# tszalay/poreseq

Measured on AMD Instinct MI355X. Metric: kb consensus refined/sec at 10x coverage, higher is better.
Workload: dtype f64; 1 GPU; poreseq consensus, 10 kb region, 10x synthetic coverage (BASELINE configs[1]), full Mutate.py schedule per region; a step is 280 independent regions per GPU = 14 lock-step batches; the batches of the timed steps run step by step (a step's batches all finish before the next step's start) through 14 batch slots (host threads) per GPU; marshalling + H2D of the events, host greedy steps and D2H inside; region_bases=10000, events=10, regions_per_gpu=280, batches_in_flight=14, step_barrier=True, parallelism=280 regions x 1 GPU(s), 14 host thread(s) per GPU, no data-path collective

## Files before the change

poreseq_amd/csrc/ps_sweep.hip:

```cpp
#include "ps_sweep_body.h"

namespace ps {

__global__ __launch_bounds__(256) void k_band(BatchD b, SweepD sw) {
    const int jd = blockIdx.y, dir = jd % sw.ndir;
    const JobD& J = b.jobs[jd / sw.ndir];
    const SweepJob& SJ = sw.sj[jd];
    const int j = blockIdx.x * 256 + threadIdx.x;
    if (j > J.C + 1) return;
    int i0 = 0, i1 = J.n0;
    if (j > J.C) { i0 = J.n0 + 1; i1 = J.n0; }
    else if (j >= 1) band_of(b.lb + J.lb_off, dir, j, J.C, J.n0, J.W, i0, i1);
    sw.band[SJ.band_off + j] = make_int2(i0, i1);
}

__global__ __launch_bounds__(256) void k_qlo(BatchD b, SweepD sw) {
    const int jd = blockIdx.y;
    const JobD& J = b.jobs[jd / sw.ndir];
    const SweepJob& SJ = sw.sj[jd];
    const int t = blockIdx.x * 256 + threadIdx.x;
    int win = 0;
    if (t < SJ.T + Q_PAD) {
        const int K = sw.K, C = J.C;
        const int2* __restrict__ band = sw.band + SJ.band_off;
        int res = -1, top = -1;
        const int qa = max(0, t - C), qb = min(SJ.Q - 1, t - 1);
        if (t < SJ.T && qa <= qb && !J.out->inert) {
            int lo = qa, hi = qb + 1;
            while (lo < hi) { const int mid = (lo + hi) >> 1; if (band[t - mid].x <= mid * K + K) hi = mid; else lo = mid + 1; }
            if (lo <= qb && band[t - lo].y >= lo * K + 1) {
                res = lo;
                int l2 = lo, h2 = qb;
                while (l2 < h2) { const int mid = (l2 + h2 + 1) >> 1; if (band[t - mid].y >= mid * K + 1) l2 = mid; else h2 = mid - 1; }
                top = l2;
                win = l2 - lo + 1;
            }
        }
        sw.qlo[SJ.q_off + t] = res;
        sw.qhi[SJ.q_off + t] = top;
    }
    for (int off = 32; off; off >>= 1) win = max(win, __shfl_xor(win, off));
    if ((threadIdx.x & 63) == 0 && win > 0) atomicMax(sw.maxwin, win);
}

#define PS_SWEEP_WPE(K) K <= 10 ? 2 : 1

template <int K, bool FD>
__global__ __launch_bounds__(64) __attribute__((amdgpu_waves_per_eu(PS_SWEEP_WPE(K), PS_SWEEP_WPE(K))))
void k_sweep(BatchD b, SweepD sw) {
    __shared__ __attribute__((aligned(16))) char mring[mring_bytes(1)];
    const JobD& J = b.jobs[blockIdx.x];
    if (J.out->inert) return;
    sweep_body<K, 1, 0, 0, FD>(b, sw, J, sw.sj[blockIdx.x], nullptr, nullptr, mring);
}

template <int K, bool FD>
__global__ __launch_bounds__(64) __attribute__((amdgpu_waves_per_eu(PS_SWEEP_WPE(K), PS_SWEEP_WPE(K))))
void k_sweep2(BatchD b, SweepD sw) {
    __shared__ unsigned long long ring[ring_cols(1)];
    __shared__ __attribute__((aligned(16))) char mring[mring_bytes(1)];
    const int jd = blockIdx.x;
    const JobD& J = b.jobs[jd >> 1];
    if (J.out->inert) return;
    if ((jd & 1) == 0) sweep_body<K, 1, 0, 1, FD>(b, sw, J, sw.sj[jd], ring, nullptr, mring);
    else sweep_body<K, 1, 1, 1, FD>(b, sw, J, sw.sj[jd], ring, nullptr, mring);
}

template <int K, bool FD>
__global__ __launch_bounds__(64) __attribute__((amdgpu_waves_per_eu(PS_SWEEP_WPE(K), PS_SWEEP_WPE(K))))
void k_sweeps(BatchD b, SweepD sw) {
    __shared__ unsigned long long ring[ring_cols(1)];
    __shared__ __attribute__((aligned(16))) char mring[mring_bytes(1)];
    const int jd = blockIdx.x;
    const JobD& J = b.jobs[jd >> 1];
    if (J.out->inert) return;
    if ((jd & 1) == 0) sweep_body<K, 1, 0, 2, FD>(b, sw, J, sw.sj[jd], ring, nullptr, mring);
    else sweep_body<K, 1, 1, 2, FD>(b, sw, J, sw.sj[jd], ring, nullptr, mring);
}

__global__ __launch_bounds__(64) void k_best(BatchD b, SweepD sw) {
    chain_priority();
    const JobD& J = b.jobs[blockIdx.x];
    JobOut* O = J.out;
    if (O->inert) return;
    const SweepJob& SJ = sw.sj[blockIdx.x * sw.ndir];
    const StripBest* SB = sw.sb + SJ.sb_off;
    double v = 0.0;
    int bi = 0x7fffffff, bj = 0x7fffffff;
    for (int q = threadIdx.x; q < SJ.Q; q += 64) {
        const StripBest s = SB[q];
        if (s.v > v || (s.v == v && s.v > 0.0 && (s.j < bj || (s.j == bj && s.i < bi)))) { v = s.v; bi = s.i; bj = s.j; }
    }
    for (int off = 32; off; off >>= 1) {
        const double ov = __shfl_xor(v, off);
        const int oi = __shfl_xor(bi, off), oj = __shfl_xor(bj, off);
        if (ov > v || (ov == v && ov > 0.0 && (oj < bj || (oj == bj && oi < bi)))) { v = ov; bi = oi; bj = oj; }
    }
    if (threadIdx.x == 0) {
        O->best = v;
        if (v > 0.0) { O->bi = bi; O->bj = bj; } else { O->bi = 0; O->bj = 0; }
    }
}

template <int K>
struct StripCodes {
    const unsigned char* codes;
    const int2* band;
    const int* st;
    int nl;
    int ci0, ci1, cp0, cp1, cst;
    static constexpr bool ROWFAST = true;
    static constexpr bool TWO_PASS = true;
    __device__ __forceinline__ void prep(int, int tj, int t) {
        const int col = tj - (t & 63);
        ci0 = 1; ci1 = 0; cp0 = 0; cp1 = -1; cst = -1;
        if (col >= 1) {
            const int2 bc = band[col], bp = band[col - 1];
            ci0 = bc.x; ci1 = bc.y; cp0 = bp.x; cp1 = bp.y; cst = st[col - 1];
        }
    }
    __device__ __forceinline__ unsigned fetch(int ti, int tj, int a, int c) const {
        const int rs = max(ti - a, 1), col = max(tj - c, 1);
        const int q = (rs - 1) / K, rr = (rs - 1) - q * K;
        return code_fetch(codes + (size_t)(col + q) * (nl * K), K, q & (nl - 1), rr, nl);
    }
    __device__ __forceinline__ unsigned short decode(unsigned by, int ti, int tj, int a, int c) const {
        const int r = ti - a;
        const int cu = __builtin_amdgcn_readfirstlane(c);
        const int i0 = __builtin_amdgcn_readlane(ci0, cu), i1 = __builtin_amdgcn_readlane(ci1, cu);
        const int p0 = __builtin_amdgcn_readlane(cp0, cu), p1 = __builtin_amdgcn_readlane(cp1, cu);
        const int sc = __builtin_amdgcn_readlane(cst, cu);
        const bool cell = r >= 1 && tj - cu >= 1 && sc >= 0 && r >= i0 && r <= i1;
        const bool vd = r > p0 && r <= p1;
        const unsigned sm = code_main_step(by, vd), ss = code_stay_step(by);
        const unsigned w = sm | (ss << 8) | ((by & CB_POS) ? 0u : 0x4000u) | ((by & CB_SPOS) ? 0u : 0x8000u);
        return (unsigned short)(cell ? w : 0xC000u);
    }
};

template <int K>
__global__ __launch_bounds__(256) void k_backtrace_s(BatchD b, SweepD sw) {
    const JobD& J = b.jobs[blockIdx.x];
    const SweepJob& SJ = sw.sj[blockIdx.x * sw.ndir];
    StripCodes<K> src;
    src.codes = sw.codes + SJ.codes_off;
    src.band = sw.band + SJ.band_off;
    src.st = J.st;
    src.nl = sw.nl;
    bt_walk(J, src);
}

template <bool FD>
__device__ __forceinline__ double cell_emission(const BatchD& b, const JobD& J, int i, int j) {
    const int state = J.st[j - 1];
    const double2* row = (const double2*)((const char*)J.model8 + (size_t)max(state, 0) * MODEL_ROW_BYTES);
    const double2 q0 = row[0], q1 = row[1], q2 = row[2], q3 = row[3];
    const double m[8] = {q0.x, q0.y, q1.x, q1.y, q2.x, q2.y, q3.x, q3.y};
    const double4 l4 = ((const double4*)J.lev[0])[i - 1];
    const double lv[4] = {l4.x, l4.y, l4.z, l4.w};
    return emission8<FD>(m, lv, b.log2pi, J.lik_offset);
}

template <bool FD>
__global__ __launch_bounds__(256) void k_like_a(BatchD b) {
    const JobD& J = b.jobs[blockIdx.y];
    if (J.out->inert) return;
    const int t = blockIdx.x * 256 + threadIdx.x;
    if (t >= J.n0) return;
    const long long w = ((const long long*)J.rl)[t];
    double o = 0.0;
    if (w != 0) {
        const int j = (int)(w >> 4), st = (int)(w >> 1) & 7;
        if (st == (int)M_MATCH || st == (int)M_STAY || st == (int)M_EXTEND) o = cell_emission<FD>(b, J, t + 1, j);
    }
    J.ri[t] = o;
}

template <bool FD>
__global__ __launch_bounds__(64) void k_like_b(BatchD b) {
    chain_priority();
    const JobD& J = b.jobs[blockIdx.x];
    const JobOut O = *J.out;
    if (O.inert || O.bi <= 0) return;
    const int lane = threadIdx.x;
    const int iz = O.term_i, jz = O.term_w >> 3, kind = O.term_w & 3;
    const double lsk = J.lsk, lst = J.lst, lex = J.lex, lin = J.lin;
    double v = 0.0;
    if ((kind & 1) && iz >= 1 && jz >= 1) v = cell_emission<FD>(b, J, iz, jz);
    int curj = jz;
    long long* rlw = (long long*)J.rl;
    for (int i0 = iz + 1; i0 <= O.bi; i0 += 64) {
        const int i = i0 + lane;
        long long w = 0; double o = 0.0;
        if (i <= O.bi) { w = rlw[i - 1]; o = J.ri[i - 1]; }
        const int wj = (int)(w >> 4), wst = (int)(w >> 1) & 7;
        double res = 0.0;
        const int n = min(64, O.bi - i0 + 1);
        for (int k = 0; k < n; k++) {
            const int j = __builtin_amdgcn_readlane(wj, k), st = __builtin_amdgcn_readlane(wst, k);
            const double ok = __hiloint2double(__builtin_amdgcn_readlane(__double2hiint(o), k), __builtin_amdgcn_readlane(__double2loint(o), k));
            const int jx = (st == (int)M_MATCH || st == (int)M_IGNORE) ? j - 1 : j;
            for (int s = curj; s < jx; s++) v = v + lsk;
            if (st == (int)M_MATCH) v = v + ok;
            else if (st == (int)M_IGNORE || st == (int)M_INSERT) v = v + lin;
            else if (st == (int)M_STAY) v = v + ok + lst;
            else v = v + ok + lex;
            curj = j;
            res = lane == k ? v : res;
        }
        if (i <= O.bi) J.rl[i - 1] = res;
    }
}

constexpr int LK_MAXC = 12 * 1024;
__global__ __launch_bounds__(256) void k_likes(BatchD b, const LikeGroup* __restrict__ groups, double* __restrict__ out) {
    __shared__ int s_idx[LK_MAXC];
    __shared__ int s_part[256];
    const LikeGroup G = groups[blockIdx.x];
    const int tid = threadIdx.x, nk = G.C + 4;
    double* __restrict__ lk = out + G.out_off;
    const int chunk = (nk + 255) / 256, k0 = min(nk, tid * chunk), k1 = min(nk, k0 + chunk);
    for (int k = tid; k < G.len; k += 256) lk[k] = 0.0;
    for (int e = 0; e < G.njobs; e++) {
        const JobD& J = b.jobs[G.job0 + e];
        const double* __restrict__ ra = J.ra;
        const double* __restrict__ rl = J.rl;
        for (int k = tid; k < nk; k += 256) s_idx[k] = -1;
        __syncthreads();
        for (int t = tid; t < J.n0; t += 256) {
            const double a = ra[t];
            if (a > 0) { const int k = (int)a; if (k < nk) atomicMax(&s_idx[k], t); }
        }
        __syncthreads();
        int run = -1;
        for (int k = k0; k < k1; k++) { run = max(run, s_idx[k]); s_idx[k] = run; }
        s_part[tid] = run;
        __syncthreads();
        int before = -1;
        for (int q = 0; q < tid; q++) before = max(before, s_part[q]);
        for (int k = k0; k < k1; k++) {
            const int t = max(s_idx[k], before);
            if (k >= 1 && k < G.C + 3 && k + 1 < G.len) lk[k + 1] += t >= 0 ? rl[t] : 0.0;
        }
        __syncthreads();
    }
}

int launch_likes(Runtime* rt, const BatchD& b, const LikeGroup* d_groups, int ngroups, double* d_out) {
    if (!ngroups) return PS_OK;
    hipLaunchKernelGGL(k_likes, dim3(ngroups), dim3(256), 0, rt->stream, b, d_groups, d_out);
    PS_LAUNCH_CHECK();
    return PS_OK;
}
int likes_max_states() { return LK_MAXC - 4; }

struct SweepHeight { int K; bool on[3]; };
static const SweepHeight HEIGHTS[] = {
#define PS_X(K, W1, W2, W4) {K, {W1, W2, W4}},
    PS_SWEEP_HEIGHTS(PS_X)
#undef PS_X
};
template <class F>
static int first_height(int NW, F ok) {
    const int c = NW == 1 ? 0 : NW == 2 ? 1 : NW == 4 ? 2 : -1;
    for (const SweepHeight& h : HEIGHTS) if (c >= 0 && h.on[c] && ok(h.K)) return h.K;
    return 0;
}
int sweep_win_max(int NW) { return 64 * NW - 1; }
int sweep_guess_window(int W, int K) { return (2 * W + 1) / (K + 1) + 3; }

SweepForm sweep_guess_form(int W, int NW) {
    SweepForm f;
    f.K = first_height(NW, [&](int K) { return sweep_guess_window(W, K) <= sweep_win_max(NW); });
    if (f.K) f.NW = NW;
    return f;
}
SweepForm sweep_next_form(SweepForm f, int win) {
    SweepForm n;
    n.K = first_height(f.NW, [&](int K) { return K > f.K; });
    if (n.K) n.NW = f.NW;
    else if (f.NW > 1) n.K = first_height(1, [&](int K) { return K * sweep_win_max(1) > f.K * win; });
    return n;
}
bool sweep_form_exists(int K, int NW) { return first_height(NW, [&](int k) { return k == K; }) != 0; }
int sweep_guess_k(int W) { return sweep_guess_form(W, 1).K; }

template <int K>
static void sweep_launch_k(Runtime* rt, const BatchD& b, const SweepD& sw) {
    if (sw.ndir == 2 && sw.sparse) with_fastdiv(b.fastdiv, [&](auto fd) { hipLaunchKernelGGL((k_sweeps<K, fd.value>), dim3(b.njobs * 2), dim3(64), 0, rt->stream, b, sw); });
    else if (sw.ndir == 2) with_fastdiv(b.fastdiv, [&](auto fd) { hipLaunchKernelGGL((k_sweep2<K, fd.value>), dim3(b.njobs * 2), dim3(64), 0, rt->stream, b, sw); });
    else with_fastdiv(b.fastdiv, [&](auto fd) { hipLaunchKernelGGL((k_sweep<K, fd.value>), dim3(b.njobs), dim3(64), 0, rt->stream, b, sw); });
}

double sweep_job_bytes(int n0, int C, SweepForm f, bool full) {
    const int K = std::max(f.K, 1);
    const double steps = (double)C + (n0 + K - 1) / K + 1;
    return steps * 64.0 * f.NW * K * (full ? 1.0 + 2 * 16.0 : 1.0);
}

int sweep_prepare(Runtime* rt, Batch& bt, SweepForm f) {
    const BatchD& b = bt.d;
    const int nd = bt.ndir, K = f.K, NL = 64 * f.NW;
    std::vector<SweepJob>& sj = bt.sjobs;
    sj.resize(bt.jobs.size() * nd);
    int64_t band_tot = 0, q_tot = 0, sb_tot = 0, code_tot = 0, rec_tot = 0;
    int maxT = 0;
    for (size_t k = 0; k < bt.jobs.size(); k++) {
        JobD& j = bt.jobs[k];
        j.K = nd == 2 ? (bt.sparse ? -1 : K) : 0;
        j.NL = NL;
        if (bt.sparse) j.pitch = (std::min(2 * j.W + 1, j.n0) + 2 * (K - 1) + 3) & ~1;
        for (int d = 0; d < nd; d++) {
            SweepJob s;
            s.Q = (j.n0 + K - 1) / K;
            s.T = j.C + s.Q;
            s.band_off = band_tot; band_tot += j.C + 2;
            s.q_off = q_tot; q_tot += s.T + Q_PAD;
            s.sb_off = sb_tot; if (d == 0) sb_tot += std::max(s.Q, 1);
            s.codes_off = code_tot; if (d == 0) code_tot += (int64_t)s.T * NL * K;
            if (nd == 2 && bt.sparse) { j.mat_off[d] = rec_tot + (K - 1); rec_tot += (int64_t)bt.nkeep[2 * k + d] * j.pitch + 2 * K; }
            else if (nd == 2) { j.mat_off[d] = rec_tot; rec_tot += (int64_t)s.T * NL * K; }
            maxT = std::max(maxT, s.T);
            sj[k * nd + d] = s;
        }
    }
    bt.sweep_K = K; bt.sweep_NW = f.NW; bt.sweep_maxT = maxT; bt.sweep_code_bytes = code_tot; bt.sweep_sb = sb_tot; bt.sweep_recs = rec_tot;
    PS_TRY(rt->buf("sw_jobs").ensure(std::max<size_t>(sj.size(), 1) * sizeof(SweepJob)));
    PS_TRY(rt->buf("sw_band").ensure(std::max<int64_t>(band_tot, 1) * sizeof(int2)));
    PS_TRY(rt->buf("sw_qlo").ensure(std::max<int64_t>(q_tot, 1) * sizeof(int)));
    PS_TRY(rt->buf("sw_qhi").ensure(std::max<int64_t>(q_tot, 1) * sizeof(int)));
    PS_TRY(rt->buf("sw_sb").ensure(std::max<int64_t>(sb_tot, 1) * sizeof(StripBest)));
    PS_TRY(rt->buf("sw_win").ensure(64));
    PS_TRY(rt->up(rt->buf("sw_jobs").p, sj.data(), sj.size() * sizeof(SweepJob)));
    SweepD& sw = bt.sd;
    sw.sj = rt->buf("sw_jobs").as<SweepJob>();
    sw.band = rt->buf("sw_band").as<int2>();
    sw.qlo = rt->buf("sw_qlo").as<int>();
    sw.qhi = rt->buf("sw_qhi").as<int>();
    sw.sb = (StripBest*)rt->buf("sw_sb").p;
    sw.maxwin = rt->buf("sw_win").as<int>();
    sw.codes = nullptr;
    sw.K = K;
    sw.nl = NL;
    sw.ndir = nd;
    sw.sparse = nd == 2 && bt.sparse ? 1 : 0;
    PS_HIP(hipMemsetAsync(sw.maxwin, 0, sizeof(int), rt->stream));
    hipLaunchKernelGGL(k_band, dim3((bt.maxC + 2 + 255) / 256, b.njobs * nd), dim3(256), 0, rt->stream, b, sw);
    hipLaunchKernelGGL(k_qlo, dim3((maxT + Q_PAD + 255) / 256, b.njobs * nd), dim3(256), 0, rt->stream, b, sw);
    PS_LAUNCH_CHECK();
    return PS_OK;
}

int sweep_run(Runtime* rt, Batch& bt) {
    const BatchD& b = bt.d;
    SweepD& sw = bt.sd;
    const int K = bt.sweep_K, NW = bt.sweep_NW;
    if (!sweep_form_exists(K, NW)) return fail(PS_ERR_BAD_ARG, "sweep_run: no strip sweep of " + std::to_string(K) + " rows per lane on " + std::to_string(NW) + " wavefronts is built");
    PS_HIP(hipMemsetAsync(sw.sb, 0, (size_t)std::max<int64_t>(bt.sweep_sb, 1) * sizeof(StripBest), rt->stream));
    prof_begin(rt);
    if (NW > 1) {
        if (!b.fastdiv || !sweepw_launch(rt, b, sw, K, NW)) return fail(PS_ERR_BAD_ARG, "sweep_run: no such multi-wavefront form");
    } else {
        switch (K) {
#define PS_X(K, W1, W2, W4) PS_FORM_##W1(case K: sweep_launch_k<K>(rt, b, sw); break;)
            PS_SWEEP_HEIGHTS(PS_X)
#undef PS_X
        }
    }
    PS_LAUNCH_CHECK();
    prof_end(rt, "sweep", 0.0);
    if (rt->prof_on) {
        if (NW > 1) rt->prof[NW == 2 ? "sweep_w2" : "sweep_w4"].launches++;
        if (bt.ndir == 2 && bt.sparse) rt->prof["sweep_kept"].launches++;
        if (!b.fastdiv) rt->prof["sweep_ieee"].launches++;
    }
    hipLaunchKernelGGL(k_best, dim3(b.njobs), dim3(64), 0, rt->stream, b, sw);
    if (bt.ndir == 2) PS_TRY(launch_prefix(rt, b, 2));
    switch (K) {
#define PS_X(K, W1, W2, W4) case K: hipLaunchKernelGGL((k_backtrace_s<K>), dim3(b.njobs), dim3(256), 0, rt->stream, b, sw); break;
        PS_SWEEP_HEIGHTS(PS_X)
#undef PS_X
    }
    PS_LAUNCH_CHECK();
    if (bt.maxn > 0) {
        with_fastdiv(b.fastdiv, [&](auto fd) {
            hipLaunchKernelGGL(k_like_a<fd.value>, dim3((bt.maxn + 255) / 256, b.njobs), dim3(256), 0, rt->stream, b);
            hipLaunchKernelGGL(k_like_b<fd.value>, dim3(b.njobs), dim3(64), 0, rt->stream, b);
        });
        PS_LAUNCH_CHECK();
    }
    return PS_OK;
}

}
```

poreseq_amd/csrc/ps_sweep_body.h:

```cpp
#ifndef PS_SWEEP_BODY_H_
#define PS_SWEEP_BODY_H_

#include "ps_dev.h"
#include "ps_host.h"
#include "ps_codes.h"

namespace ps {

#ifdef __HIPCC__
__device__ __forceinline__ unsigned code_push(unsigned w, bool c) {
    const unsigned long long m = __builtin_amdgcn_ballot_w64(c);
    unsigned long long carry_out;
    asm("v_addc_co_u32_e64 %0, %1, %2, %2, %3" : "=v"(w), "=s"(carry_out) : "v"(w), "s"(m));
    return w;
}
__device__ __forceinline__ unsigned code_first(bool c) {
    const unsigned long long m = __builtin_amdgcn_ballot_w64(c);
    unsigned w;
    asm("v_cndmask_b32_e64 %0, 0, 1, %1" : "=v"(w) : "s"(m));
    return w;
}
#endif

struct StripBest { double v; int i, j; };
constexpr int Q_PAD = 8;

__device__ __forceinline__ double wave_ror1(double v) {
    int lo = __double2loint(v), hi = __double2hiint(v);
    lo = __builtin_amdgcn_update_dpp(lo, lo, 0x13C , 0xf, 0xf, false);
    hi = __builtin_amdgcn_update_dpp(hi, hi, 0x13C, 0xf, 0xf, false);
    return __hiloint2double(hi, lo);
}

__host__ __device__ constexpr int mring_slots(int nw) { return 128 * nw; }
__host__ __device__ constexpr int mring_bytes(int nw) { return (mring_slots(nw) + 1) * MODEL_ROW_BYTES; }

__host__ __device__ constexpr int ring_cols(int nw) { return nw <= 2 ? 256 : 512; }
constexpr int HAND_DOUBLES = 4;

template <int K, int NW, int DIR, int MODE, bool FD>
__device__ __forceinline__ void sweep_body(const BatchD& b, const SweepD& sw, const JobD& J, const SweepJob& SJ, unsigned long long* ring, double* hand, char* mring) {
    constexpr int NL = 64 * NW;
    constexpr int RING = ring_cols(NW);
    constexpr int RM = mring_slots(NW);
    const int lane = threadIdx.x;
    const int wv = NW > 1 ? uni((int)threadIdx.x >> 6) : 0;
    const int C = uni(J.C), T = uni(SJ.T), n0 = uni(J.n0);
    typedef const __attribute__((address_space(4))) int* kcip;
    kcip QLO = (kcip)uni_ptr(sw.qlo + SJ.q_off);
    kcip QHI = (kcip)uni_ptr(sw.qhi + SJ.q_off);
    gcip band = (gcip)uni_ptr((const int*)(sw.band + SJ.band_off));
    gcip st = (gcip)uni_ptr(J.st);
    const PS_GLOBAL char* model = (const PS_GLOBAL char*)uni_ptr((const char*)J.model8);
    const PS_GLOBAL v4d* levs = (const PS_GLOBAL v4d*)uni_ptr(J.lev[DIR]);
    PS_GLOBAL unsigned char* codes = (PS_GLOBAL unsigned char*)uni_ptr(sw.codes + SJ.codes_off);
    PS_GLOBAL char* rec = (PS_GLOBAL char*)uni_ptr((char*)(b.rec + J.mat_off[DIR]));
    PS_GLOBAL double* gcmax = (PS_GLOBAL double*)uni_ptr(b.cmax + J.col_off[DIR]);
    StripBest* SB = sw.sb + SJ.sb_off;
    const double lsk = J.lsk, lst = J.lst, lex = J.lex, lin = J.lin, off = J.lik_offset, log2pi = b.log2pi;
    const double NINF = -__builtin_inf();

    struct Ahead { int p1, i0, i1, sc, kc, ro; };
    gcip keep = (gcip)uni_ptr(J.keep[DIR]);
    const int pitch = uni(J.pitch);
    const PS_GLOBAL char* band_c = (const PS_GLOBAL char*)band;
    const PS_GLOBAL char* st_c = (const PS_GLOBAL char*)(DIR == 0 ? st - 1 : st);
    const PS_GLOBAL char* keep_c = (const PS_GLOBAL char*)keep;
    const PS_GLOBAL char* levs_c = (const PS_GLOBAL char*)levs;
    auto fetch = [&](int tt, int ql) -> Ahead {
        const int q = ql + ((lane - ql) & (NL - 1));
        const int j = clampi(tt - q, 1, max(C, 1));
        Ahead a;
        typedef int v3i_a4 __attribute__((ext_vector_type(3), aligned(4)));
        const v3i_a4 b3 = *(const PS_GLOBAL v3i_a4*)(band_c + (unsigned)(8 * j - 4));
        a.p1 = b3.x; a.i0 = b3.y; a.i1 = b3.z;
        a.sc = *(const PS_GLOBAL int*)(st_c + (unsigned)(4 * (DIR == 0 ? j : C - j)));
        a.kc = MODE == 2 ? *(const PS_GLOBAL int*)(keep_c + (unsigned)(4 * j)) : -1;
        a.ro = (j & (RM - 1)) * MODEL_ROW_BYTES;
        return a;
    };
    auto model_row = [&](const Ahead& a, double (&m)[8]) {
        const v2d* row = (const v2d*)(mring + a.ro);
        const v2d q0 = row[0], q1 = row[1], q2 = row[2], q3 = row[3];
        m[0] = q0.x; m[1] = q0.y; m[2] = q1.x; m[3] = q1.y; m[4] = q2.x; m[5] = q2.y; m[6] = q3.x; m[7] = q3.y;
    };

    const bool feeder = wv == 0;
    typedef const __attribute__((address_space(4))) int* kst_t;
    kst_t st_k = (kst_t)uni_ptr(J.st);
    int jf = 0;
    int fs0 = -1, fs1 = -1, fsb = -1;
    auto st_of = [&](int c) -> int { return st_k[DIR == 0 ? c - 1 : C - c]; };
    auto ring_at = [&](int c, int q16) -> v4i* { return (v4i*)(mring + (c <= C ? (c & (RM - 1)) : RM) * MODEL_ROW_BYTES + q16); };
    auto feed_now = [&](int hi) {
        const int fcol = (lane & 63) >> 2, fq16 = (lane & 3) * 16;
        const int lo = max(1, hi - (NL - 2));
        if (jf < lo - 1) jf = lo - 1;
        while (jf < hi) {
            const int c = jf + 1 + fcol, cc = min(c, max(C, 1));
            const int state = *(const PS_GLOBAL int*)(st_c + (unsigned)(4 * (DIR == 0 ? cc : C - cc)));
            const v4i row = *(const PS_GLOBAL v4i*)(model + (unsigned)max(state, 0) * (unsigned)MODEL_ROW_BYTES + (unsigned)fq16);
            *ring_at(c, fq16) = row;
            jf += 16;
        }
        fsb = -1;
    };
    v4i frow = {0, 0, 0, 0};
    bool fput = false;
    auto f_top = [&](int hi_next, int jn_now) {
        if (!feeder) return;
        if (hi_next > 0 && jf < min(C, hi_next)) feed_now(min(C, hi_next));
        fput = false;
        if (jf < C && fsb == jf && jn_now > 0 && jf + 2 <= jn_now + NL + 1) {
            if ((lane & 63) < 8) {
                const int state = (lane & 4) ? fs1 : fs0;
                frow = *(const PS_GLOBAL v4i*)(model + (unsigned)max(state, 0) * (unsigned)MODEL_ROW_BYTES + (unsigned)((lane & 3) * 16));
            }
            fput = true;
        }
    };
    auto f_end = [&]() {
        if (!feeder) return;
        if (fput) {
            if ((lane & 63) < 8) *ring_at(jf + 1 + ((lane & 4) >> 2), (lane & 3) * 16) = frow;
            jf += 2;
        }
        if (jf < C && fsb != jf) { fsb = jf; fs0 = st_of(min(jf + 1, C)); fs1 = st_of(min(jf + 2, C)); }
    };

    double lev[K][4];
    double pm[K];
    double pe[DIR ? K : 1];
#pragma unroll
    for (int r = 0; r < K; r++) { pm[r] = NINF; if (DIR) pe[r] = NINF; lev[r][0] = 0.0; lev[r][1] = 1.0; lev[r][2] = 0.0; lev[r][3] = 1.0; }
    int qcur = -1;
    double bot_m = NINF, bot_s = NINF, bot_e = NINF;
    double dm = NINF, de = NINF;
    double lbest = 0.0;
    int lbt = 0, lbr = 0;
    int flushed = 1, next_flush = 64;
    if (MODE) {
        for (int k = lane; k < RING; k += NL) ring[k] = 0ull;
    }
    const int pw = NW > 1 ? (wv + NW - 1) % NW : 0;
    const bool l0 = NW > 1 && (lane & 63) == 0, l63 = NW > 1 && (lane & 63) == 63;
    if (NW > 1) {
        if (l63) {
#pragma unroll
            for (int s = 0; s < 2; s++) { double* h = hand + (s * NW + wv) * HAND_DOUBLES; h[0] = NINF; h[1] = NINF; h[2] = NINF; }
        }
        asm volatile("s_waitcnt lgkmcnt(0)\n\ts_barrier" ::: "memory");
    }

    int ql0 = QLO[1], ql1 = QLO[2], ql2 = QLO[3];
    Ahead aA = fetch(1, ql0), aB = fetch(2, ql1), aC = aB;
    double mr[8];
    if (feeder) { feed_now(min(max(C, 1), ql0 >= 0 ? max(1 - ql0, 1) : 1)); if (jf < C) { fsb = jf; fs0 = st_of(min(jf + 1, C)); fs1 = st_of(min(jf + 2, C)); } }
    if (NW > 1) asm volatile("s_waitcnt lgkmcnt(0)\n\ts_barrier" ::: "memory");
    model_row(aA, mr);
    int qlev = -1;
    auto load_levels = [&](int ql_next) {
        if (ql_next < 0) return;
        const int qn = ql_next + ((lane - ql_next) & (NL - 1));
        if (qn != qlev) {
            qlev = qn;
#pragma unroll
            for (int r = 0; r < K; r++) {
                const v4d v = *(const PS_GLOBAL v4d*)(levs_c + (unsigned)(32 * min(qn * K + r, n0 - 1)));
                lev[r][0] = v.x; lev[r][1] = v.y; lev[r][2] = v.z; lev[r][3] = v.w;
            }
        }
    };
    load_levels(ql0);

    constexpr bool DEFER_REC = MODE == 2 && K <= 5;
    bool pend = false;
    unsigned cwp[(K + 3) / 4];
    double pnm[DEFER_REC ? K : 1], pns[DEFER_REC ? K : 1];
    bool pkept = false;
    unsigned poff = 0u;
#pragma unroll
    for (int w = 0; w < (K + 3) / 4; w++) cwp[w] = 0u;
    auto put_codes = [&](int tp, const unsigned (&cw)[(K + 3) / 4]) {
        PS_GLOBAL unsigned char* dst = codes + (size_t)tp * (NL * K);
        int r0 = 0;
#pragma unroll
        for (int g = 0; g < 8; g++) {
            const int sz = plane_sz(K - r0);
            PS_GLOBAL unsigned char* p = dst + (unsigned)(NL * r0 + lane * sz);
            if (sz == 16) {
                v4i v;
                v.x = cw[r0 / 4]; v.y = cw[r0 / 4 + 1]; v.z = cw[r0 / 4 + 2]; v.w = cw[r0 / 4 + 3];
                *(PS_GLOBAL v4i*)p = v;
            } else if (sz == 8) {
                typedef int v2i __attribute__((ext_vector_type(2)));
                v2i v;
                v.x = cw[r0 / 4]; v.y = cw[r0 / 4 + 1];
                *(PS_GLOBAL v2i*)p = v;
            } else if (sz == 4) {
                *(PS_GLOBAL unsigned*)p = cw[r0 / 4];
            } else {
                const int nrow = K - (r0 & ~3) < 4 ? K - (r0 & ~3) : 4;
                const int sh = CODE_BITS * (nrow - (r0 & 3) - sz);
                if (sz == 2) *(PS_GLOBAL unsigned short*)p = (unsigned short)(cw[r0 / 4] >> sh);
                else *p = (unsigned char)(cw[r0 / 4] >> sh);
            }
            r0 += sz;
            if (r0 >= K) break;
        }
    };
    auto put_pending = [&](int tp) {
        if (!pend) return;
        if (DIR == 0) put_codes(tp, cwp);
        if (DEFER_REC) {
            if (pkept) {
                PS_GLOBAL char* recp = rec - 16 * (K - 1) + poff;
#pragma unroll
                for (int r = 0; r < K; r++) *(PS_GLOBAL v2d*)(recp + r * 16) = (v2d){pnm[r], pns[r]};
            }
        }
    };

    auto step = [&](const int t, const Ahead& a0, const Ahead& a1, Ahead& a2) __attribute__((always_inline)) {
        const int ql = ql0;
        const bool live = ql >= 0;
        const int q = ql + ((lane - ql) & (NL - 1));
        const int j = t - q;
        if (live && q != qcur) {
            if (DIR == 0 && lbest > 0.0) { StripBest sbv; sbv.v = lbest; sbv.i = qcur * K + 1 + lbr; sbv.j = lbt - qcur; SB[qcur] = sbv; }
            lbest = 0.0;
            qcur = q;
#pragma unroll
            for (int r = 0; r < K; r++) { pm[r] = NINF; if (DIR) pe[r] = NINF; }
        }
        f_top(ql1 >= 0 ? t + 1 - ql1 : 0, ql >= 0 ? t - ql : 0);
        a2 = fetch(t + 2, ql2);
        __builtin_amdgcn_sched_barrier(0);
        double ov[K];
#pragma unroll
        for (int r = 0; r < K; r++) {
            ov[r] = emission8<FD>(mr, lev[r], log2pi, off);
            asm volatile("" : "+v"(ov[r]));
            if (r & 1) __builtin_amdgcn_sched_barrier(0);
        }
        __builtin_amdgcn_sched_barrier(0);
        double hm = NINF, hs = NINF, he = NINF;
        if (NW > 1) {
            asm volatile("s_waitcnt lgkmcnt(0)\n\ts_barrier" ::: "memory");
            const double* h = hand + (((t - 1) & 1) * NW + pw) * HAND_DOUBLES;
            const v2d hv = *(const v2d*)h;
            hm = hv.x; hs = hv.y;
            if (DIR) he = h[2];
        }
        put_pending(t - 1);
        load_levels(ql1);
        model_row(a1, mr);
        const int ql3 = QLO[t + 3];
        pend = live;
        if (MODE != 1 || live) {
            const int base = q * K + 1;
            const bool valid = live && j >= 1 && j <= C && a0.sc >= 0;
            const int ra = valid ? a0.i0 - base : K, rb = valid ? a0.i1 - base : -1;
            const int rp = a0.p1 - base;
            double um = wave_ror1(bot_m), us = wave_ror1(bot_s), ue = DIR ? wave_ror1(bot_e) : 0.0;
            if (NW > 1) { um = l0 ? hm : um; us = l0 ? hs : us; if (DIR) ue = l0 ? he : ue; }
            double dprev = dm, deprev = de;
            dm = um; de = ue;
            const double lbefore = lbest;
            double crun = 0.0;
            PS_GLOBAL char* recp = rec + ((size_t)t * K * NL + lane) * 16;
            const bool kept = MODE == 2 && live && a0.kc >= 0 && j >= 1 && j <= C;
            const bool kstore = kept && ra < K && rb >= 0;
            if (MODE == 2) {
                const unsigned ro = (unsigned)((a0.kc * pitch + (base - a0.i0) + (K - 1)) * 16);
                recp = rec - 16 * (K - 1) + ro;
                if (DEFER_REC) { poff = ro; pkept = kstore; }
                if (kept && !valid)
                    for (int r = max(0, a0.i0 - base); r <= min(K - 1, a0.i1 - base); r++) *(PS_GLOBAL v2d*)(recp + (size_t)r * 16) = (v2d){0.0, 0.0};
            }
            unsigned cw = 0u;
#pragma unroll
            for (int r = 0; r < K; r++) {
                const double o = ov[r];
                const bool act = r >= ra && r <= rb;
                const bool top = r == ra;
                const bool below = r - 1 >= ra && r <= rb;
                const double pmr = pm[r];
                double L;
                asm("v_max_f64 %0, %1, 0" : "=v"(L) : "v"(pmr));
                const bool blank = rp == r - 1;
                const double dq = __hiloint2double(blank ? (int)0xFFEFFFFF : __double2hiint(dprev), __double2loint(dprev));
                double D = dq;
                if (DIR == 0) asm("v_max_f64 %0, %1, 0" : "=v"(D) : "v"(dq));
                const double eq_ = DIR ? __hiloint2double(blank ? (int)0xFFEFFFFF : __double2hiint(deprev), __double2loint(deprev)) : 0.0;
                const double cSTAY = DIR == 0 ? um + o + lst : ue + lst;
                const double cEXT = DIR == 0 ? us + o + lex : us + lex;
                const double cINS = um + lin;
                const double cSKIP = L + lsk;
                const double cMATCH = DIR == 0 ? D + o : eq_;
                const double cIGN = dq + lin;
                const double floor_s = MODE == 1 ? (top ? -BIG : 0.0) : 0.0;
                const double t1 = fmax(floor_s, cSTAY);
                const double ns = fmax(t1, cEXT);
                double nm = fmax(0.0, cSKIP);
                nm = fmax(nm, cMATCH);
                nm = fmax(nm, cINS);
                nm = fmax(nm, cIGN);
                nm = fmax(nm, ns);
                if (DIR == 0) {
                    cw = (r & 3) == 0 ? code_first(cEXT > t1) : code_push(cw, cEXT > t1);
                    cw = code_push(cw, ns > 0.0);
                    cw = code_push(cw, cSKIP == nm);
                    cw = code_push(cw, cMATCH == nm);
                    cw = code_push(cw, cINS == nm);
                    cw = code_push(cw, cIGN == nm);
                    cw = code_push(cw, nm > 0.0);
                    if ((r & 3) == 3 || r == K - 1) cwp[r >> 2] = cw;
                }
                const double nmx = keep_or_absent(nm, act), nsx = keep_or_absent(ns, MODE == 1 ? act : below);
                dprev = pmr;
                pm[r] = nmx;
                if (DIR) { deprev = pe[r]; pe[r] = nmx + o; }
                um = nmx;
                us = DIR == 0 ? nsx : nsx + o;
                if (DIR) ue = nmx + o;
                if (MODE == 1) {
                    double rx;
                    asm("v_max_f64 %0, %1, 0" : "=v"(rx) : "v"(nmx));
                    *(PS_GLOBAL v2d*)(recp + (size_t)r * (16 * NL)) = (v2d){rx, act ? ns : 0.0};
                    crun = fmax(crun, rx);
                }
                if (MODE == 2) {
                    if (DEFER_REC) { pnm[r] = nmx; pns[r] = nsx; }
                    else if (kstore) *(PS_GLOBAL v2d*)(recp + r * 16) = (v2d){nmx, nsx};
                    crun = fmax(crun, nmx);
                }
                if (DIR == 0) {
                    const bool gt = nmx > lbest;
                    asm("v_max_f64 %0, %1, %2" : "=v"(lbest) : "v"(lbest), "v"(nmx));
                    lbr = gt ? r : lbr;
                }
                __builtin_amdgcn_sched_barrier(0);
            }
            bot_m = um; bot_s = us; bot_e = ue;
            if (DIR == 0) lbt = lbest > lbefore ? t : lbt;
            if (MODE) atomicMax(&ring[(unsigned)j & (RING - 1)], (unsigned long long)__double_as_longlong(crun));
            if (MODE && live && t >= next_flush) {
                const int jdone = min(t - QHI[t], C + 1);
                for (int col = flushed + lane; col < jdone; col += NL) {
                    unsigned long long* e = &ring[(unsigned)col & (RING - 1)];
                    const unsigned long long v = *e;
                    *e = 0ull;
                    gcmax[col] = __longlong_as_double((long long)v);
                }
                flushed = max(flushed, jdone);
                next_flush = t + 64;
            }
        } else {
            bot_m = NINF; bot_s = NINF; bot_e = NINF;
        }
        if (NW > 1 && l63) {
            double* h = hand + ((t & 1) * NW + wv) * HAND_DOUBLES;
            *(v2d*)h = (v2d){bot_m, bot_s};
            if (DIR) h[2] = bot_e;
        }
        f_end();
        ql0 = ql1; ql1 = ql2; ql2 = ql3;
    };

    constexpr int UNROLL_MAXK = 5;
    if (K <= UNROLL_MAXK) {
        for (int t = 1; t < T; t += 3) {
            step(t, aA, aB, aC);
            step(t + 1, aB, aC, aA);
            step(t + 2, aC, aA, aB);
        }
        put_pending(T - 1 + (3 - (T - 1) % 3) % 3);
    } else {
        for (int t = 1; t < T; t++) {
            step(t, aA, aB, aC);
            aA = aB; aB = aC;
        }
        put_pending(T - 1);
    }
    if (DIR == 0 && qcur >= 0 && lbest > 0.0) { StripBest sbv; sbv.v = lbest; sbv.i = qcur * K + 1 + lbr; sbv.j = lbt - qcur; SB[qcur] = sbv; }
    if (NW > 1 && MODE) asm volatile("s_waitcnt lgkmcnt(0)\n\ts_barrier" ::: "memory");
    if (MODE)
        for (int col = flushed + lane; col <= C; col += NL) gcmax[col] = __longlong_as_double((long long)ring[(unsigned)col & (RING - 1)]);
}

bool sweepw_launch(Runtime* rt, const BatchD& b, const SweepD& sw, int K, int NW);

}
#endif
```

Measured before the change: 224.1 kb/s.

## Stage per-column band/state/keep records in the LDS model ring via feeder wave

Moves the per-lane per-step global gathers of band bounds, state and keep index into the feeder wave, which writes a packed 16-byte column record into the LDS model ring next to each model row. The compute step then reads that record from LDS instead of issuing scattered global loads two steps ahead. This shortens the software pipeline from three to two steps and adds a window check for the lane that falls outside the fed range. The packing caps state count and sequence length, so a host-side fit check is added, and the codes buffer is padded by two steps. The cost is extra LDS writes by the feeder and some extra feeder global loads.

```diff
diff --git a/poreseq_amd/csrc/ps_colrec.h b/poreseq_amd/csrc/ps_colrec.h
--- /dev/null
+++ b/poreseq_amd/csrc/ps_colrec.h
@@ -0,0 +1,29 @@
+#ifndef PS_COLREC_H_
+#define PS_COLREC_H_
+
+#if defined(__HIPCC__)
+#define PS_COLREC_FN __host__ __device__
+#else
+#define PS_COLREC_FN
+#endif
+
+namespace ps {
+
+constexpr int COLREC_BYTES = 16;
+constexpr int COLREC_SC_BITS = 11;
+constexpr unsigned COLREC_SC_MASK = (1u << COLREC_SC_BITS) - 1u;
+constexpr int COLREC_SC_MAX = (int)COLREC_SC_MASK - 1;
+constexpr int COLREC_KC_MAX = (int)((1u << (32 - COLREC_SC_BITS)) - 2u);
+
+PS_COLREC_FN inline unsigned colrec_pack(int sc, int kc) {
+    return (sc < 0 ? 0u : (unsigned)sc + 1u) | ((kc < 0 ? 0u : (unsigned)kc + 1u) << COLREC_SC_BITS);
+}
+PS_COLREC_FN inline int colrec_sc(unsigned w) { return (int)(w & COLREC_SC_MASK) - 1; }
+PS_COLREC_FN inline int colrec_kc(unsigned w) { return (int)(w >> COLREC_SC_BITS) - 1; }
+
+PS_COLREC_FN inline bool colrec_fits(int n_states, long long C) {
+    return n_states >= 0 && n_states - 1 <= COLREC_SC_MAX && C >= 0 && C + 1 <= (long long)COLREC_KC_MAX;
+}
+
+}
+#endif
diff --git a/poreseq_amd/csrc/ps_sweep.hip b/poreseq_amd/csrc/ps_sweep.hip
--- a/poreseq_amd/csrc/ps_sweep.hip
+++ b/poreseq_amd/csrc/ps_sweep.hip
@@ -309,6 +309,7 @@
         JobD& j = bt.jobs[k];
         j.K = nd == 2 ? (bt.sparse ? -1 : K) : 0;
         j.NL = NL;
+        if (!colrec_fits(NS, j.C)) return fail(PS_ERR_UNSUPPORTED, "sweep_prepare: a sequence of " + std::to_string(j.C) + " 5-mers does not fit the strip sweep's column record (at most " + std::to_string(COLREC_KC_MAX - 1) + ")");
         if (bt.sparse) j.pitch = (std::min(2 * j.W + 1, j.n0) + 2 * (K - 1) + 3) & ~1;
         for (int d = 0; d < nd; d++) {
             SweepJob s;
@@ -317,7 +318,7 @@
             s.band_off = band_tot; band_tot += j.C + 2;
             s.q_off = q_tot; q_tot += s.T + Q_PAD;
             s.sb_off = sb_tot; if (d == 0) sb_tot += std::max(s.Q, 1);
-            s.codes_off = code_tot; if (d == 0) code_tot += (int64_t)s.T * NL * K;
+            s.codes_off = code_tot; if (d == 0) code_tot += (int64_t)(s.T + 2) * NL * K;
             if (nd == 2 && bt.sparse) { j.mat_off[d] = rec_tot + (K - 1); rec_tot += (int64_t)bt.nkeep[2 * k + d] * j.pitch + 2 * K; }
             else if (nd == 2) { j.mat_off[d] = rec_tot; rec_tot += (int64_t)s.T * NL * K; }
             maxT = std::max(maxT, s.T);
diff --git a/poreseq_amd/csrc/ps_sweep_body.h b/poreseq_amd/csrc/ps_sweep_body.h
--- a/poreseq_amd/csrc/ps_sweep_body.h
+++ b/poreseq_amd/csrc/ps_sweep_body.h
@@ -4,6 +4,7 @@
 #include "ps_dev.h"
 #include "ps_host.h"
 #include "ps_codes.h"
+#include "ps_colrec.h"
 
 namespace ps {
 
@@ -60,29 +61,34 @@
     const double lsk = J.lsk, lst = J.lst, lex = J.lex, lin = J.lin, off = J.lik_offset, log2pi = b.log2pi;
     const double NINF = -__builtin_inf();
 
-    struct Ahead { int p1, i0, i1, sc, kc, ro; };
+    struct Col { int p1, i0, i1, sc, kc; };
     gcip keep = (gcip)uni_ptr(J.keep[DIR]);
     const int pitch = uni(J.pitch);
     const PS_GLOBAL char* band_c = (const PS_GLOBAL char*)band;
     const PS_GLOBAL char* st_c = (const PS_GLOBAL char*)(DIR == 0 ? st - 1 : st);
     const PS_GLOBAL char* keep_c = (const PS_GLOBAL char*)keep;
     const PS_GLOBAL char* levs_c = (const PS_GLOBAL char*)levs;
-    auto fetch = [&](int tt, int ql) -> Ahead {
+    auto slot_of = [&](int tt, int ql) -> int {
         const int q = ql + ((lane - ql) & (NL - 1));
         const int j = clampi(tt - q, 1, max(C, 1));
-        Ahead a;
-        typedef int v3i_a4 __attribute__((ext_vector_type(3), aligned(4)));
-        const v3i_a4 b3 = *(const PS_GLOBAL v3i_a4*)(band_c + (unsigned)(8 * j - 4));
-        a.p1 = b3.x; a.i0 = b3.y; a.i1 = b3.z;
-        a.sc = *(const PS_GLOBAL int*)(st_c + (unsigned)(4 * (DIR == 0 ? j : C - j)));
-        a.kc = MODE == 2 ? *(const PS_GLOBAL int*)(keep_c + (unsigned)(4 * j)) : -1;
-        a.ro = (j & (RM - 1)) * MODEL_ROW_BYTES;
-        return a;
-    };
-    auto model_row = [&](const Ahead& a, double (&m)[8]) {
-        const v2d* row = (const v2d*)(mring + a.ro);
+        return (j & (RM - 1)) * MODEL_ROW_BYTES;
+    };
+    auto col_rec = [&](int ro) -> Col {
+        const v4i r = *(const v4i*)(mring + ro + 8 * (int)sizeof(double));
+        Col c;
+        c.p1 = r.x; c.i0 = r.y; c.i1 = r.z; c.sc = colrec_sc((unsigned)r.w); c.kc = MODE == 2 ? colrec_kc((unsigned)r.w) : -1;
+        return c;
+    };
+    auto model_row = [&](int ro, double (&m)[8]) {
+        const v2d* row = (const v2d*)(mring + ro);
         const v2d q0 = row[0], q1 = row[1], q2 = row[2], q3 = row[3];
         m[0] = q0.x; m[1] = q0.y; m[2] = q1.x; m[3] = q1.y; m[4] = q2.x; m[5] = q2.y; m[6] = q3.x; m[7] = q3.y;
+    };
+    typedef int v3i_a4 __attribute__((ext_vector_type(3), aligned(4)));
+    auto rec_load = [&](int cc, int& kc) -> v4i {
+        const v3i_a4 b3 = *(const PS_GLOBAL v3i_a4*)(band_c + (unsigned)(8 * cc - 4));
+        if (MODE == 2) kc = *(const PS_GLOBAL int*)(keep_c + (unsigned)(4 * cc));
+        return (v4i){b3.x, b3.y, b3.z, 0};
     };
 
     const bool feeder = wv == 0;
@@ -101,28 +107,45 @@
             const int state = *(const PS_GLOBAL int*)(st_c + (unsigned)(4 * (DIR == 0 ? cc : C - cc)));
             const v4i row = *(const PS_GLOBAL v4i*)(model + (unsigned)max(state, 0) * (unsigned)MODEL_ROW_BYTES + (unsigned)fq16);
             *ring_at(c, fq16) = row;
+            if ((lane & 3) == 0) {
+                int kc = -1;
+                v4i r = rec_load(cc, kc);
+                r.w = (int)colrec_pack(state, kc);
+                *ring_at(c, 8 * (int)sizeof(double)) = r;
+            }
             jf += 16;
         }
         fsb = -1;
     };
     v4i frow = {0, 0, 0, 0};
+    int fkc = -1;
     bool fput = false;
-    auto f_top = [&](int hi_next, int jn_now) {
+    auto f_top = [&](int hi_next) {
         if (!feeder) return;
         if (hi_next > 0 && jf < min(C, hi_next)) feed_now(min(C, hi_next));
+    };
+    auto f_load = [&](int jn_now) {
+        if (!feeder) return;
         fput = false;
         if (jf < C && fsb == jf && jn_now > 0 && jf + 2 <= jn_now + NL + 1) {
-            if ((lane & 63) < 8) {
-                const int state = (lane & 4) ? fs1 : fs0;
-                frow = *(const PS_GLOBAL v4i*)(model + (unsigned)max(state, 0) * (unsigned)MODEL_ROW_BYTES + (unsigned)((lane & 3) * 16));
-            }
+            typedef int v4i_a4 __attribute__((ext_vector_type(4), aligned(4)));
+            const int state = (lane & 4) ? fs1 : fs0;
+            const int cc = min(jf + 1 + (lane & 1), C);
+            const PS_GLOBAL char* src = lane < 8 ? model + ((unsigned)max(state, 0) * (unsigned)MODEL_ROW_BYTES + (unsigned)((lane & 3) * 16))
+                                                 : band_c + (unsigned)(8 * cc - 4);
+            frow = *(const PS_GLOBAL v4i_a4*)src;
+            if (MODE == 2) fkc = *(const PS_GLOBAL int*)(keep_c + (unsigned)(4 * cc));
             fput = true;
         }
     };
     auto f_end = [&]() {
         if (!feeder) return;
         if (fput) {
-            if ((lane & 63) < 8) *ring_at(jf + 1 + ((lane & 4) >> 2), (lane & 3) * 16) = frow;
+            if (lane < 8) *ring_at(jf + 1 + ((lane & 4) >> 2), (lane & 3) * 16) = frow;
+            else if (lane < 10) {
+                frow.w = (int)colrec_pack((lane & 1) ? fs1 : fs0, fkc);
+                *ring_at(jf + 1 + (lane & 1), 8 * (int)sizeof(double)) = frow;
+            }
             jf += 2;
         }
         if (jf < C && fsb != jf) { fsb = jf; fs0 = st_of(min(jf + 1, C)); fs1 = st_of(min(jf + 2, C)); }
@@ -152,12 +175,12 @@
         asm volatile("s_waitcnt lgkmcnt(0)\n\ts_barrier" ::: "memory");
     }
 
-    int ql0 = QLO[1], ql1 = QLO[2], ql2 = QLO[3];
-    Ahead aA = fetch(1, ql0), aB = fetch(2, ql1), aC = aB;
+    int ql0 = QLO[1], ql1 = QLO[2];
+    int ro0 = slot_of(1, ql0);
     double mr[8];
     if (feeder) { feed_now(min(max(C, 1), ql0 >= 0 ? max(1 - ql0, 1) : 1)); if (jf < C) { fsb = jf; fs0 = st_of(min(jf + 1, C)); fs1 = st_of(min(jf + 2, C)); } }
     if (NW > 1) asm volatile("s_waitcnt lgkmcnt(0)\n\ts_barrier" ::: "memory");
-    model_row(aA, mr);
+    model_row(ro0, mr);
     int qlev = -1;
     auto load_levels = [&](int ql_next) {
         if (ql_next < 0) return;
@@ -172,6 +195,7 @@
         }
     };
     load_levels(ql0);
+    __builtin_amdgcn_s_waitcnt(0x0F70);
 
     constexpr bool DEFER_REC = MODE == 2 && K <= 5;
     bool pend = false;
@@ -210,10 +234,9 @@
         }
     };
     auto put_pending = [&](int tp) {
-        if (!pend) return;
         if (DIR == 0) put_codes(tp, cwp);
         if (DEFER_REC) {
-            if (pkept) {
+            if (pend && pkept) {
                 PS_GLOBAL char* recp = rec - 16 * (K - 1) + poff;
 #pragma unroll
                 for (int r = 0; r < K; r++) *(PS_GLOBAL v2d*)(recp + r * 16) = (v2d){pnm[r], pns[r]};
@@ -221,11 +244,13 @@
         }
     };
 
-    auto step = [&](const int t, const Ahead& a0, const Ahead& a1, Ahead& a2) __attribute__((always_inline)) {
+    auto step = [&](const int t) __attribute__((always_inline)) {
         const int ql = ql0;
         const bool live = ql >= 0;
         const int q = ql + ((lane - ql) & (NL - 1));
         const int j = t - q;
+        const bool inwin = q - ql != NL - 1;
+        const Col a0 = col_rec(ro0);
         if (live && q != qcur) {
             if (DIR == 0 && lbest > 0.0) { StripBest sbv; sbv.v = lbest; sbv.i = qcur * K + 1 + lbr; sbv.j = lbt - qcur; SB[qcur] = sbv; }
             lbest = 0.0;
@@ -233,8 +258,7 @@
 #pragma unroll
             for (int r = 0; r < K; r++) { pm[r] = NINF; if (DIR) pe[r] = NINF; }
         }
-        f_top(ql1 >= 0 ? t + 1 - ql1 : 0, ql >= 0 ? t - ql : 0);
-        a2 = fetch(t + 2, ql2);
+        f_top(ql1 >= 0 ? t + 1 - ql1 : 0);
         __builtin_amdgcn_sched_barrier(0);
         double ov[K];
 #pragma unroll
@@ -244,6 +268,7 @@
             if (r & 1) __builtin_amdgcn_sched_barrier(0);
         }
         __builtin_amdgcn_sched_barrier(0);
+        f_load(ql >= 0 ? t - ql : 0);
         double hm = NINF, hs = NINF, he = NINF;
         if (NW > 1) {
             asm volatile("s_waitcnt lgkmcnt(0)\n\ts_barrier" ::: "memory");
@@ -252,14 +277,15 @@
             hm = hv.x; hs = hv.y;
             if (DIR) he = h[2];
         }
+        load_levels(ql1);
         put_pending(t - 1);
-        load_levels(ql1);
-        model_row(a1, mr);
-        const int ql3 = QLO[t + 3];
+        const int ro1 = slot_of(t + 1, ql1);
+        model_row(ro1, mr);
+        const int qln = QLO[t + 2];
         pend = live;
         if (MODE != 1 || live) {
             const int base = q * K + 1;
-            const bool valid = live && j >= 1 && j <= C && a0.sc >= 0;
+            const bool valid = live && inwin && j >= 1 && j <= C && a0.sc >= 0;
             const int ra = valid ? a0.i0 - base : K, rb = valid ? a0.i1 - base : -1;
             const int rp = a0.p1 - base;
             double um = wave_ror1(bot_m), us = wave_ror1(bot_s), ue = DIR ? wave_ror1(bot_e) : 0.0;
@@ -269,7 +295,7 @@
             const double lbefore = lbest;
             double crun = 0.0;
             PS_GLOBAL char* recp = rec + ((size_t)t * K * NL + lane) * 16;
-            const bool kept = MODE == 2 && live && a0.kc >= 0 && j >= 1 && j <= C;
+            const bool kept = MODE == 2 && live && inwin && a0.kc >= 0 && j >= 1 && j <= C;
             const bool kstore = kept && ra < K && rb >= 0;
             if (MODE == 2) {
                 const unsigned ro = (unsigned)((a0.kc * pitch + (base - a0.i0) + (K - 1)) * 16);
@@ -365,23 +391,21 @@
             if (DIR) h[2] = bot_e;
         }
         f_end();
-        ql0 = ql1; ql1 = ql2; ql2 = ql3;
+        ql0 = ql1; ql1 = qln; ro0 = ro1;
     };
 
     constexpr int UNROLL_MAXK = 5;
     if (K <= UNROLL_MAXK) {
-        for (int t = 1; t < T; t += 3) {
-            step(t, aA, aB, aC);
-            step(t + 1, aB, aC, aA);
-            step(t + 2, aC, aA, aB);
-        }
-        put_pending(T - 1 + (3 - (T - 1) % 3) % 3);
+        int t = 1;
+        for (; t < T; t += 3) {
+            step(t);
+            step(t + 1);
+            step(t + 2);
+        }
+        if (T >= 1) put_pending(t - 1);
     } else {
-        for (int t = 1; t < T; t++) {
-            step(t, aA, aB, aC);
-            aA = aB; aB = aC;
-        }
-        put_pending(T - 1);
+        for (int t = 1; t < T; t++) step(t);
+        if (T >= 1) put_pending(T - 1);
     }
     if (DIR == 0 && qcur >= 0 && lbest > 0.0) { StripBest sbv; sbv.v = lbest; sbv.i = qcur * K + 1 + lbr; sbv.j = lbt - qcur; SB[qcur] = sbv; }
     if (NW > 1 && MODE) asm volatile("s_waitcnt lgkmcnt(0)\n\ts_barrier" ::: "memory");
```

After: 223.0 kb/s. About the same (-0.5%).
